# facebookresearch/gtn

Measured on AMD Instinct MI355X. Metric: CTC forward+backward losses/sec (T=1000, C=256), higher is better.
Workload: dtype f32; 1 GPU; BASELINE config C3: compose(ctc_target, emissions)+forwardScore CTC loss fwd+bwd, T=1000, C=256, U=100, batch=512 per GPU; global_batch=512, parallelism=dp1 (utterance sharding, all_gather of losses), rccl_ranks=0

## Files before the change

### gtn_amd/_capi.py

```python
import ctypes as C
import os

c_graph = C.c_void_p
c_graph_p = C.POINTER(C.c_void_p)
c_i32_p = C.POINTER(C.c_int)
c_i64_p = C.POINTER(C.c_int64)
c_u8_p = C.POINTER(C.c_uint8)
c_f32_p = C.POINTER(C.c_float)

GRAD_FN = C.CFUNCTYPE(C.c_int, C.c_void_p, c_graph_p, C.c_int, c_graph)
CTX_FREE = C.CFUNCTYPE(None, C.c_void_p)

OK, INVALID_ARGUMENT, LOGIC_ERROR, RUNTIME_ERROR, OUT_OF_RANGE, DEVICE_ERROR = range(6)

_SIGS = {
    "gtnx_set_device": [C.c_int],
    "gtnx_get_device": [c_i32_p],
    "gtnx_set_stream": [C.c_void_p],
    "gtnx_compose_mode": [C.c_int, C.POINTER(C.c_int)],
    "gtnx_synchronize": [],
    "gtnx_memory_stats": [C.POINTER(C.c_uint64), C.POINTER(C.c_uint64)],
    "gtnx_empty_cache": [],
    "gtnx_reclaim": [],
    "gtnx_graph_create": [C.c_int, c_graph_p],
# ... 67 lines not shown
    "gtnx_viterbi_path_n": [c_graph_p, C.c_int, c_graph_p],
    "gtnx_items_n": [c_graph_p, C.c_int, C.c_void_p],
    "gtnx_items_device_n": [c_graph_p, C.c_int, C.c_void_p],
    "gtnx_grads_device_n": [c_graph_p, C.c_int, C.c_void_p, C.c_void_p],
    "gtnx_grads_bind_device_n": [c_graph_p, C.c_int, C.c_void_p, C.c_void_p],
    "gtnx_clone": [c_graph, C.c_int, c_graph_p],
    "gtnx_concat": [c_graph_p, C.c_int, c_graph_p],
    "gtnx_closure": [c_graph, c_graph_p],
    "gtnx_union": [c_graph_p, C.c_int, c_graph_p],
    "gtnx_batch_from_graphs": [c_graph_p, C.c_int, c_graph_p],
    "gtnx_batch_ctc_targets": [C.c_void_p, C.c_void_p, C.c_int, C.c_int, C.c_int, c_graph_p],
    "gtnx_batch_ctc_loss_step": [C.c_void_p, C.c_void_p, C.c_void_p, C.c_int, C.c_int, C.c_int, C.c_int, C.c_void_p,
                                 C.c_void_p, C.c_int, C.c_void_p],
    "gtnx_batch_ctc_loss_step_ok": [C.c_void_p, C.c_void_p, C.c_int, C.c_int, C.c_int, C.c_int, C.c_void_p, C.c_void_p,
                                    C.POINTER(C.c_int)],
    "gtnx_batch_asg_force_align": [C.c_void_p, C.c_void_p, C.c_int, c_graph, C.c_int, c_graph_p],
    "gtnx_batch_linear": [C.c_int, C.c_int, C.c_int, C.c_int, C.c_void_p, C.c_int, c_graph_p],
    "gtnx_batch_linear_rows": [C.c_int, C.c_int, C.c_int, C.c_void_p, C.c_int, C.c_void_p, C.c_int, c_graph_p],
    "gtnx_batch_destroy": [c_graph],
    "gtnx_batch_size": [c_graph, c_i32_p],
    "gtnx_batch_get": [c_graph, C.c_int, c_graph_p],
    "gtnx_batch_negate": [c_graph, c_graph_p],
    "gtnx_batch_add": [c_graph, c_graph, c_graph_p],
    "gtnx_batch_subtract": [c_graph, c_graph, c_graph_p],
    "gtnx_batch_subtract_into": [c_graph, c_graph, C.c_void_p, c_graph_p],
    "gtnx_batch_compose": [c_graph, c_graph, c_graph_p],
    "gtnx_batch_intersect": [c_graph, c_graph, c_graph_p],
    "gtnx_batch_forward_score": [c_graph, c_graph_p],
    "gtnx_batch_viterbi_score": [c_graph, c_graph_p],
    "gtnx_batch_viterbi_path": [c_graph, c_graph_p],
# ... 137 lines not shown
```

### gtn_amd/csrc/band_backward_body.inc

```
  constexpr int RNk = K >= 4 ? 4 : K;
  constexpr int NP = K / RNk;
  const BandPair P = GTNX_BAND_PAIR;
  const int T = P.T, C = P.C, NS = P.NS;
  extern __shared__ float lds[];
  const BandLds L = band_lds(C, K, NSmax, true);
  float* ering = lds + L.o_ering;
  float* aring = lds + L.o_aring;
  float* oring = lds + L.o_oring;
  int* snode = reinterpret_cast<int*>(lds + L.o_snode);
  const BandMisc M = band_misc<K>(lds, L);
  float* lser = M.lsep;
  const int CS = L.CS;
  const int wv = __builtin_amdgcn_readfirstlane(threadIdx.x >> 6);
  const bool sweeper = wv < 4;
  const int l = threadIdx.x & 63;
  const int nblocks = (T + K - 1) / K;
  const int nticks = nblocks + 5;
  const GTNX_G double* ao = P.aoff;
  const double z2 = uniform(ao[0]);
  const bool dead = !(z2 > double(DEADF));
  const float ds = uniform(P.delta[0]);
  const bool want_em = P.grad_em != nullptr;
  GTNX_TM_INIT(128);
  constexpr bool SPLIT = !BIG && K >= 2 && GTNX_BWD_SPLIT;
// ... 121 lines not shown
    const bool have = all != 0.0f && !dead_r;
    const float f = have ? ds * __builtin_amdgcn_rcpf(all) : 1.0f;
    if ((l & 15) == 15 && (STEADY || (l >> 4) < rows)) {
      if (P.hot >= 0) {
        const float sm = dn_k * ex2(em_hot - ls_hot);
        const GTNX_G char* gb = reinterpret_cast<const GTNX_G char*>(P.grad_em + int64_t(T - c * K - K) * C);
        *reinterpret_cast<GTNX_G float*>(const_cast<GTNX_G char*>(gb) + unsigned(4 * R.go)) = (dead_r ? 0.0f : hotp * f) + sm;
      }
      rnorm_k[cg * K + (l >> 4)] = f;
    }
  };
  constexpr int NCS = 8 / K;
  struct DrainRegs {
    int s[NCS], e[NCS], n0[NCS], n1[NCS];
    float m0[NCS], m1[NCS];
    bool more_any;
  };
  auto drain_init = [&](DrainRegs& D, int hid) {
    const int* cls = reinterpret_cast<const int*>(oring);
#pragma unroll
    for (int q = 0; q < NCS; ++q) {
      const int cc = hid + q * BW;
      D.s[q] = D.e[q] = 0;
      if (cc < C && cc != P.hot) {
        D.s[q] = cls[cc];
        D.e[q] = cls[C + cc];
      }
      const int cnt = D.e[q] - D.s[q];
      D.n0[q] = cnt > 0 ? snode[D.s[q]] : 0;
      D.n1[q] = cnt > 1 ? snode[D.s[q] + 1] : 0;
      D.m0[q] = cnt > 0 ? 1.0f : 0.0f;
      D.m1[q] = cnt > 1 ? 1.0f : 0.0f;
    }
    D.more_any = false;
#pragma unroll
    for (int q = 0; q < NCS; ++q) D.more_any = D.more_any || __builtin_amdgcn_ballot_w64(D.e[q] - D.s[q] > 2) != 0;
  };
  auto drain_rows = [&](const DrainRegs& D, int hid, int c, int cg , auto full_tag, auto dead_tag, auto r0_tag, auto r1_tag) {
    constexpr bool FULL = decltype(full_tag)::value;
    constexpr bool DEADU = decltype(dead_tag)::value;
    constexpr int R0 = decltype(r0_tag)::value, R1 = decltype(r1_tag)::value;
    const int rows = FULL ? K : rows_of_k(c);
    const float* ob = oring + cg * K * NSmax;
    const float* eb = ering + ge_of(c) * K * CS;
    const float* lb = lser + cg * K;
    const float* fb = rnorm_k + cg * K;
    GTNX_G float* dst = P.grad_em + int64_t(T - 1 - c * K) * C;
#pragma unroll
    for (int q = 0; q < NCS; ++q) {
      if (q > 0 && q * BW >= C) break;
      const int cc = hid + q * BW;
      const bool mine = cc < C && cc != P.hot;
      float p0[K], p1[K], e[K], ls[K], f[K];
#pragma unroll
      for (int r = R0; r < R1; ++r) {
        if constexpr (!DEADU) {
          p0[r] = ob[r * NSmax + D.n0[q]];
          p1[r] = ob[r * NSmax + D.n1[q]];
        }
        e[r] = eb[r * CS + min(cc, C - 1)];
      }
      if constexpr (K == 4) {
        const gtnx_f4 l4 = *reinterpret_cast<const gtnx_f4*>(lb), f4 = *reinterpret_cast<const gtnx_f4*>(fb);
        ls[0] = l4.x, ls[1] = l4.y, ls[2] = l4.z, ls[3] = l4.w;
        f[0] = f4.x, f[1] = f4.y, f[2] = f4.z, f[3] = f4.w;
      } else {
#pragma unroll
        for (int r = R0; r < R1; ++r) {
          ls[r] = lb[r];
          f[r] = fb[r];
        }
      }
      float sum[K];
      if constexpr (!DEADU) {
#pragma unroll
      for (int r = R0; r < R1; ++r) sum[r] = p0[r] * D.m0[q] + p1[r] * D.m1[q];
      }
      if (!DEADU && D.more_any) {
        for (int i = D.s[q] + 2; i < D.e[q]; ++i) {
          const float* o = ob + snode[i];
#pragma unroll
          for (int r = R0; r < R1; ++r) sum[r] += o[r * NSmax];
        }
      }
      float val[K];
#pragma unroll
      for (int r = R0; r < R1; ++r) {
        const float sm = dn_k * ex2(e[r] - ls[r]);
        val[r] = DEADU ? sm : sum[r] * f[r] + sm;
      }
      if (mine) {
#pragma unroll
        for (int r = R0; r < R1; ++r) {
          if (FULL || r < rows) {
            GTNX_G float* row = dst - int64_t(r) * C;
            row[cc] = val[r];
          }
        }
      }
    }
  };
  auto drain_block = [&](const DrainRegs& D, int hid, int c, int cg, auto r0_tag, auto r1_tag) {
    if (!want_em || c >= nblocks) return;
    if (dead) drain_rows(D, hid, c, cg, std::false_type{}, std::true_type{}, r0_tag, r1_tag);
    else if (c * K + K <= T) drain_rows(D, hid, c, cg, std::true_type{}, std::false_type{}, r0_tag, r1_tag);
    else drain_rows(D, hid, c, cg, std::false_type{}, std::false_type{}, r0_tag, r1_tag);
  };
  constexpr int KH = SPLIT ? K / 2 : K;

  if (sweeper) {
#ifndef GTNX_BWD_SWEEP_PRIO
#define GTNX_BWD_SWEEP_PRIO 1
#endif
    __builtin_amdgcn_s_setprio(GTNX_BWD_SWEEP_PRIO);
    const int w = wv;
    const int lag = 3 - w;
    const int m0 = threadIdx.x * NPL;
    NodeRegs<NPL> g;
    load_nodes<NPL, true>(P, m0, g);
    float b[NPL], post[NPL], acc[3][NPL];
    const double Ahi = uniform(ao[1 + (T >> P.lgrn) * 4 + w]);
// ... 14 lines not shown
    }
    float* bnd_own = M.bndr + (4 - w) * 4 * K * 2;
    const float* bnd_prev = M.bndr + (3 - w) * 4 * K * 2;
    double* off_own = M.offr + (4 - w) * 16;
    const double* off_prev = M.offr + (3 - w) * 16;
    if (threadIdx.x < 8 * K) M.bndr[threadIdx.x] = NEGF;
    if (threadIdx.x < 16) M.offr[threadIdx.x] = 0.0;
    if (l == 0) off_own[0] = 0.0;
    lds_barrier();
    lds_barrier();
    RowSumRegs rsr;
    if constexpr (!SPLIT && !RS4) rowsum_init(rsr);
    float gscale = ds;
    int bm5 = ring_start(-lag, NBE), bm7 = ring_start(-lag, NBG), rm7 = ring_start(RS4 ? -5 : -4, NBG);
    lds_barrier();
    auto tick = [&](int tau, auto steady_tag) {
      constexpr bool STEADY = decltype(steady_tag)::value;
      GTNX_TM(0);
      if constexpr (RS4) {
#ifndef GTNX_EXP_NO_GSCALE
        if (GRADG && want_em && (STEADY || (tau >= 5 && (tau - 5) * K + K <= T))) gscale = rnorm_k[rm7 * K + w];
#endif
      } else if constexpr (!SPLIT) {
#ifndef GTNX_EXP_NO_ROWSUM
        if (STEADY || tau >= 4) {
          const float fr = rowsum_do(rsr, tau - 4, rm7, w, steady_tag);
#ifndef GTNX_EXP_NO_GSCALE
          if (fr != 0.0f) gscale = fr;
#endif
        }
// ... 134 lines not shown
        }
        if (NPL == 1 ? l < 2 : l == 0) {
#pragma unroll
          for (int i = 0; i < K; ++i)
            if (FULL || i < rows) {
              float* bp = bnd_own + ((beta & 3) * K + i) * 2;
              if (NPL == 1) {
                bp[l] = qh[i][0];
              } else {
                bp[0] = qh[i][0];
                bp[1] = qh[i][NPL - 1];
              }
            }
        }
      };
      if constexpr (STEADY) {
        block(std::true_type{});
      } else if (beta >= 0 && beta < nblocks && !dead) {
        if (beta * K + K <= T) block(std::true_type{});
        else block(std::false_type{});
      }
      GTNX_TM(5);
      lds_barrier();
      GTNX_TM(6);
      GTNX_TM_TICK();
    };
    {
      const int s0 = min(RS4 ? 5 : 4, nticks), s1 = dead ? s0 : max(s0, min(nticks, T / K + lag));
      auto step_rings = [&]() { ring_step(bm5, NBE), ring_step(bm7, NBG), ring_step(rm7, NBG); };
      int tau = 0;
      for (; tau < s0; ++tau, step_rings()) tick(tau, std::false_type{});
      for (; tau < s1; ++tau, step_rings()) tick(tau, std::true_type{});
      for (; tau < nticks; ++tau, step_rings()) tick(tau, std::false_type{});
    }
    GTNX_TM_DUMP();
    if (GRADG && P.grad_fixed) {
#pragma unroll
      for (int j = 0; j < NPL; ++j)
#pragma unroll
        for (int k = 0; k < 3; ++k)
          if (g.ao[k][j] >= 0) P.grad_fixed[g.ao[k][j]] = dead ? 0.0f : acc[k][j];
    }
  } else if (wv < 8) {
    const bool soft = P.delta_norm != nullptr && P.rowlse != nullptr;
    lds_barrier();
    if constexpr (!BIG) {
      const int h = wv - 4, q = h & 1;
      auto rows_of = [&](int c) { return c < nblocks ? min(K, T - c * K) : 0; };
      auto tlo_of = [&](int c) { return T - c * K - rows_of(c); };
      DrainRegs dr_s;
      const int hid_s = threadIdx.x - BW;
      auto drain_upper = [&](int tau) {
        if constexpr (SPLIT) {
          if (tau >= 5) drain_block(dr_s, hid_s, tau - 5, (tau - 5) % NBG, std::integral_constant<int, KH>{}, std::integral_constant<int, K>{});
        }
      };
      if (h < 2) {
        Stage<16, 64> se;
        if constexpr (VEC) se.init_offsets(C, CS, K, l);
        auto issue_em = [&](int c, auto steady_tag) {
          constexpr bool ST = decltype(steady_tag)::value;
          const int rows = ST ? K : rows_of(c);
          se.template issue<VEC>(P.em + int64_t(T - c * K - rows) * C, rows * C, l);
        };
        auto land_em = [&](int c, auto steady_tag) {
          constexpr bool ST = decltype(steady_tag)::value;
          const int rows = ST ? K : rows_of(c);
          se.settle_all();
          GTNX_TM(4);
// ... 5 lines not shown
              const f2v lo = f2v{v4.x, v4.y} * LOG2E, hi = f2v{v4.z, v4.w} * LOG2E;
              *reinterpret_cast<gtnx_f4*>(eb + o) = gtnx_f4{fmaxf(lo.x, NEGF), fmaxf(lo.y, NEGF), fmaxf(hi.x, NEGF), fmaxf(hi.y, NEGF)};
            });
          } else {
            se.template each<false>(rows * C, C, l, [&](int, int, int r, int col, gtnx_f4 v4) {
              eb[(rows - 1 - r) * CS + col] = em2(v4.x);
            });
          }
        };
        issue_em(q, std::false_type{});
        land_em(q, std::false_type{});
        issue_em(q + 2, std::false_type{});
        RowSum4Regs rs4;
        if constexpr (RS4) rowsum4_init(rs4);
        lds_barrier();
        if constexpr (SPLIT) drain_init(dr_s, hid_s);
        lds_barrier();
        int r7 = ring_start(-4, NBG);
        auto tick = [&](int tau, auto steady_tag) {
          constexpr bool ST = decltype(steady_tag)::value;
          GTNX_TM(0);
#ifndef GTNX_EXP_NO_STAGE
          if (((tau + 2) & 1) == q) {
            land_em(tau + 2, steady_tag);
            GTNX_TM(1);
            issue_em(tau + 4, steady_tag);
            GTNX_TM(2);
          } else if constexpr (RS4) {
#ifndef GTNX_EXP_NO_ROWSUM
            if (ST || tau >= 4) rowsum4_do(rs4, tau - 4, r7, steady_tag);
#endif
// ... 31 lines not shown
          const int rows = ST ? K : rows_of(c);
          sa.settle_all();
          asm volatile("" : "+v"(lse_s), "+v"(af_s));
          if (rows <= 0) return;
          float* ab = aring + c5 * K * NSmax;
          sa.each_vec(rows * NS, (K - rows) * NSmax, l, [&](int, int o, gtnx_f4 v4) { *reinterpret_cast<gtnx_f4*>(ab + o) = v4; });
          if (l < rows) lser[c7 * K + rows - 1 - l] = lse_s;
          if (l < 4 * rows) M.aofr[(c5 * K) * 4 + l] = af_s;
        };
        issue_rest(q, std::false_type{});
        if (q == 0) {
          land_rest(0, 0, 0, std::false_type{});
          issue_rest(2, std::false_type{});
        }
        lds_barrier();
        if constexpr (SPLIT) drain_init(dr_s, hid_s);
        lds_barrier();
        int s5 = ring_start(1, NBE), s7 = ring_start(1, NBG);
        auto tick = [&](int tau, auto steady_tag) {
          GTNX_TM(0);
#ifndef GTNX_EXP_NO_STAGE
          if (((tau + 1) & 1) == q) {
            land_rest(tau + 1, s5, s7, steady_tag);
            GTNX_TM(1);
            issue_rest(tau + 3, steady_tag);
            GTNX_TM(2);
          }
#endif
          drain_upper(tau);
          GTNX_TM(3);
          lds_barrier();
// ... 86 lines not shown
    GTNX_TM_DUMP();
    }
  } else {
    const int hid = threadIdx.x - 2 * BW;
    const bool soft = P.delta_norm != nullptr && P.rowlse != nullptr;
    int* cls = reinterpret_cast<int*>(oring);
    for (int c = hid; c < 2 * C; c += BW) cls[c] = 0;
    lds_barrier();
    for (int i = hid; i < P.n_lab; i += BW) {
      const int lab = P.slab[i];
      snode[i] = P.snode[i];
      if (i == 0 || P.slab[i - 1] != lab) cls[lab] = i;
      if (i == P.n_lab - 1 || P.slab[i + 1] != lab) cls[C + lab] = i + 1;
    }
    lds_barrier();
    DrainRegs dr;
    drain_init(dr, hid);
    RowSumRegs rsr;
    if constexpr (SPLIT) rowsum_init(rsr);
    const int dw = wv - 8;
    lds_barrier();
    int d7 = ring_start(-5, NBG);
    for (int tau = 0; tau < nticks; ++tau, ring_step(d7, NBG)) {
      GTNX_TM(0);
#ifndef GTNX_EXP_NO_DRAIN
      if (tau >= 5) drain_block(dr, hid, tau - 5, d7, std::integral_constant<int, 0>{}, std::integral_constant<int, KH>{});
#endif
      if constexpr (SPLIT) {
        if (tau >= 4) rowsum_do(rsr, tau - 4, (tau - 4) % NBG, dw, std::false_type{});
      }
      GTNX_TM(3);
      lds_barrier();
      GTNX_TM(6);
      GTNX_TM_TICK();
    }
    GTNX_TM_DUMP();
  }
```

### gtn_amd/csrc/band_forward_body.inc

```
#ifndef GTNX_FWD_SHIFT_ROWS
#define GTNX_FWD_SHIFT_ROWS 4
#endif
  constexpr int RNk = K >= GTNX_FWD_SHIFT_ROWS ? GTNX_FWD_SHIFT_ROWS : (K >= 4 ? 4 : K);
  constexpr int NP = K / RNk;
  constexpr int D = 8 / K > GTNX_FWD_DEPTH ? 8 / K : GTNX_FWD_DEPTH;
  const BandPair P = GTNX_BAND_PAIR;
  const int T = P.T, C = P.C, NS = P.NS;
  extern __shared__ float lds[];
  const BandLds L = band_lds(C, K, NSmax, false);
  float* ering = lds + L.o_ering;
  const BandMisc M = band_misc<K>(lds, L);
  const int CS = L.CS;
  const int wv = __builtin_amdgcn_readfirstlane(threadIdx.x >> 6);
  const bool sweeper = wv < 4;
  const int l = threadIdx.x & 63;
  const int nblocks = (T + K - 1) / K;
  const int nticks = nblocks + 3;
  GTNX_TM_INIT(0);

  if (sweeper) {
    __builtin_amdgcn_s_setprio(1);
    const int w = wv;
    const int m0 = threadIdx.x * NPL;
    NodeRegs<NPL> g;
// ... 16 lines not shown
    const double* off_prev = M.offr + w * 16;
    if (threadIdx.x < 8 * K) M.bndr[threadIdx.x] = NEGF;
    if (threadIdx.x < 16) M.offr[threadIdx.x] = 0.0;
    if (l == 0) {
      P.aoff[1 + w] = 0.0;
      off_own[0] = 0.0;
    }
    if (NPL == 1) {
      if (l >= 62) bnd_own[63 - l] = a[0];
    } else if (l == 63) {
      bnd_own[0] = a[NPL - 1];
      bnd_own[1] = a[0];
    }
    lds_barrier();
    int bm5 = ((-w % NBE) + NBE) % NBE;
    for (int tau = 0; tau < nticks; ++tau, bm5 = bm5 + 1 == NBE ? 0 : bm5 + 1) {
      GTNX_TM(0);
      const int beta = tau - w;
      auto block = [&](auto full_tag) {
        constexpr bool FULL = decltype(full_tag)::value;
        const int t0 = beta * K, rows = FULL ? K : min(K, T - t0);
        const float* eb = ering + bm5 * K * CS;
        float ev[K][NPL], bv1[K], bv2[K];
        double offp[NP + 1];
#pragma unroll
        for (int i = 0; i < K; ++i) {
#pragma unroll
#ifdef GTNX_EXP_NOCONFLICT
          for (int j = 0; j < NPL; ++j) ev[i][j] = eb[i * CS + l * NPL + j];
#else
          for (int j = 0; j < NPL; ++j) ev[i][j] = eb[i * CS + g.lab[j]];
// ... 298 lines not shown
```

### gtn_amd/csrc/batch.cpp

```cpp
#include "batch.h"

#include <algorithm>
#include <atomic>
#include <cstdlib>
#include <cstring>
#include <limits>
#include <unordered_map>
#include <unordered_set>

namespace gtnx {

namespace {

std::atomic<uint64_t> g_batch_seq{1};

struct CompMode {
  int old;
  CompMode() : old(compose_mode_hint(2)) {}
  ~CompMode() { compose_mode_hint(old); }
};

BatchP make_batch(Batch::Kind k, int n, bool cg) {
  auto b = std::make_shared<Batch>();
  b->kind = k;
  b->n = n;
  b->calc_grad = cg;
  return b;
}

// ... 540 lines not shown
  d.aoff = arena->as<double>(o_aoff);
  d.rowlse = arena->as<float>(o_lse);
  d.score = arena->as<float>(o_score);
  d.norm = arena->as<float>(o_norm);
  d.em_stride = int64_t(T) * C;
  d.rec_stride = int64_t(rec_stride);
  d.alpha_stride = int64_t(alpha_stride);
  d.aoff_stride = int64_t(aoff_stride);
  d.o_flags = int(o_flags);
  d.o_snode = int(o_snode);
  d.o_slab = int(o_slab);
  d.T = T;
  d.C = C;
  d.blank = blank;
  d.lgrn = band_forward_lgrn(C);
  {
    GTNX_PROF("band_forward_score_grad", bytes);
    launch_ctc_step(d, n, max_ns, target_grad, rt.stream());
  }
}


BatchP batch_asg_force_align(const int* labels, const int* lengths, int n, Graph& transitions, int n_labels) {
  if (n < 0) throw_invalid("[gtnx_batch_asg_force_align] negative batch size");
  if (transitions.num_nodes() != int64_t(n_labels) + 1 || transitions.num_arcs() != int64_t(n_labels) * (n_labels + 1))
    throw_invalid("[gtnx_batch_asg_force_align] the transitions graph must have the asgTransitions(N) layout");
  BatchP b = make_batch(Batch::CTC_TARGETS, n, transitions.calc_grad());
  b->fal = true;
  b->trans = transitions;
  b->trans_labels = n_labels;
// ... 499 lines not shown
    std::shared_ptr<PendingCopy> pend = ch.w_pend;
    std::unique_lock<std::mutex> pend_lock;
    bool fuse_copy = false;
    if (pend && !pend->done.load(std::memory_order_acquire)) {
      pend_lock = std::unique_lock<std::mutex>(pend->mu);
      fuse_copy = !pend->done.load(std::memory_order_relaxed) && pend->device == rt.device();
      const size_t A = size_t(T) * size_t(C);
      for (int b = 0; b < n && fuse_copy; ++b) fuse_copy = pend->src_of(ch.w_dev + size_t(b) * A) != nullptr;
      fuse_copy = fuse_copy && pend->segs.size() == size_t(n);
      if (!fuse_copy) {
        pend_lock.unlock();
        pend->settle();
      }
    }
    int64_t goff_run = 0;
    for (int b = 0; b < n; ++b) {
      BandPair& p = op->pairs[size_t(b)];
      p = BandPair{};
      const int U = fx.lab_off[size_t(b) + 1] - fx.lab_off[size_t(b)];
      const size_t N = fx.fal ? size_t(U) + 1 : size_t(2 * U + 1);
      char* base = fx.rec_mem->as<char>(fx.rec_off[size_t(b)]);
      p.nodes = reinterpret_cast<BandNode*>(base);
      base += align_up(sizeof(BandNode) * N, 64);
      p.nflags = reinterpret_cast<uint8_t*>(base);
      base += align_up(N, 64);
      p.snode = reinterpret_cast<int*>(base);
      base += align_up(4 * N, 64);
      p.slab = reinterpret_cast<int*>(base);
      p.n_lab = fx.fal ? U : int(N);
      p.w = fx.fal ? fx.rec_mem->as<float>(fx.w_off[size_t(b)]) : nullptr;
      p.em = ch.w_dev + size_t(b) * size_t(T) * size_t(C);
      p.N = int(N);
      p.T = ch.rows_of(b);
      p.C = C;
      p.NS = band_row_stride(p.N, band_npl(p.N));
      p.alpha = op->arena->as<float>(ao[size_t(b)]);
      p.aoff = op->arena->as<double>(oo[size_t(b)]);
      p.score = op->arena->as<float>(4 * size_t(b));
      if (want_norm) {
        p.norm = op->arena->as<float>(o_norm + 4 * size_t(b));
        p.rowlse = op->arena->as<float>(o_lse + 4 * size_t(b) * size_t(T));
      }
      p.hot = (!fx.fal && U + 1 >= 8) ? fx.blank : -1;
      p.lgrn = band_forward_lgrn(C);
      p.bidx = b;
      p.goff = goff_run;
      goff_run += int64_t(fx.elem_size(b));
      BandPair q = p;
      if (fuse_copy) {
        q.em = static_cast<const float*>(pend->src_of(p.em));
        q.em_copy = const_cast<float*>(p.em);
      }
      tab.push_back({BandLaunchKey{C, band_npl(q.N), fx.fal ? 0 : 1, 0, band_vec_ok(q)}, q});
      abytes += 4.0 * p.T * C + 4.0 * double(p.T + 1) * p.NS + (fuse_copy ? 4.0 * T * C : 0.0);
    }
    band_launch(tab, false, "band_forward_score", abytes, fuse_copy ? nullptr : &op->fwd_table);
    if (fuse_copy) pend->done.store(true, std::memory_order_release);
    if (want_norm) {
      ch.nc_mem = op->arena;
// ... 296 lines not shown
```

### gtn_amd/csrc/capi.cpp

```cpp
#include <atomic>
#include <chrono>
#include <condition_variable>
#include <cstdlib>
#include <cstring>
#include <mutex>
#include <string>
#include <vector>

#include "batch.h"
#include "lm_graph.h"
#include "ops.h"
#include "ops_internal.h"
#include "region.h"

#define GTNX_API extern "C" __attribute__((visibility("default")))

using namespace gtnx;

namespace {
thread_local std::string g_err;

gtnx_status_t fail(gtnx_status_t s, const std::string& m) {
  g_err = m;
  return s;
// ... 745 lines not shown
}
GTNX_API gtnx_status_t gtnx_batch_ctc_loss_step(const void* emissions, const int* labels, const int* lengths, int n, int T,
                                                int C, int blank, void* loss, void* grad, int target_grad,
                                                void* target_grad_dev) {
  return guard([&] {
    batch_ctc_loss_step(emissions, labels, lengths, n, T, C, blank, loss, grad, target_grad != 0, target_grad_dev);
  });
}
GTNX_API gtnx_status_t gtnx_batch_ctc_loss_step_ok(const int* labels, const int* lengths, int n, int T, int C, int blank,
                                                   const void* emissions, const void* grad, int* ok) {
  return guard([&] {
    if (!ok) throw_invalid("[gtnx_batch_ctc_loss_step_ok] null result pointer");
    *ok = ctc_step_fused_ok(labels, lengths, n, T, C, blank, emissions, grad) ? 1 : 0;
  });
}
GTNX_API gtnx_status_t gtnx_batch_asg_force_align(const int* labels, const int* lengths, int n, gtnx_graph_t transitions,
                                                  int n_labels, gtnx_batch_t* out) {
  return guard([&] { *out = HB(batch_asg_force_align(labels, lengths, n, G(transitions), n_labels)); });
}
GTNX_API gtnx_status_t gtnx_batch_linear(int n, int M, int N, int cg, const void* dev, int borrow, gtnx_batch_t* out) {
  return guard([&] { *out = HB(batch_linear(n, M, N, cg != 0, dev, borrow != 0)); });
}
GTNX_API gtnx_status_t gtnx_batch_linear_rows(int n, int M, int N, const int* rows, int cg, const void* dev, int borrow,
                                             gtnx_batch_t* out) {
  return guard([&] { *out = HB(batch_linear(n, M, N, cg != 0, dev, borrow != 0, rows)); });
}
GTNX_API gtnx_status_t gtnx_batch_destroy(gtnx_batch_t b) {
  return guard([&] {
    auto* p = reinterpret_cast<BatchP*>(b);
    if (!p) return;
// ... 477 lines not shown
```

### gtn_amd/csrc/ctc_step.hip

```cpp
#include <hip/hip_runtime.h>

#include <algorithm>
#include <atomic>
#include <stdexcept>
#include <type_traits>

#include "kernels.h"

namespace gtnx {
namespace {

#include "band_device.inc"

__device__ float g_ctc_step_seeds[2] = {-1.0f, 1.0f};

__device__ __forceinline__ BandPair step_pair(const CtcStepDesc& d, int b, const gtnx_i4 e) {
  BandPair P;
  const int U = e.y, N = 2 * U + 1;
  GTNX_G char* rec = reinterpret_cast<GTNX_G char*>(d.rec) + int64_t(b) * d.rec_stride;
  P.nodes = reinterpret_cast<const GTNX_G BandNode*>(rec);
  P.nflags = reinterpret_cast<const GTNX_G uint8_t*>(rec + d.o_flags);
  P.snode = reinterpret_cast<const GTNX_G int*>(rec + d.o_snode);
  P.slab = reinterpret_cast<const GTNX_G int*>(rec + d.o_slab);
  P.w = nullptr;
// ... 5 lines not shown
  P.rowlse = reinterpret_cast<GTNX_G float*>(d.rowlse) + int64_t(b) * d.T;
  P.norm = reinterpret_cast<GTNX_G float*>(d.norm) + b;
  P.delta = (const GTNX_G float*)g_ctc_step_seeds;
  P.delta_norm = (const GTNX_G float*)(g_ctc_step_seeds + 1);
  P.grad_em = reinterpret_cast<GTNX_G float*>(d.grad) + int64_t(b) * d.em_stride;
  P.grad_fixed = d.tgrad ? reinterpret_cast<GTNX_G float*>(d.tgrad) + e.w : nullptr;
  P.N = N;
  P.T = e.z;
  P.C = d.C;
  P.NS = (N + 3) & ~3;
  P.hot = U + 1 >= 8 ? d.blank : -1;
  P.lgrn = d.lgrn;
  P.n_lab = N;
  P.bidx = b;
  P.goff = e.w;
  return P;
}

__device__ __forceinline__ BandPair uniform_pair(const BandPair& s) {
  constexpr int NW = int(sizeof(BandPair) / 4);
  static_assert(sizeof(BandPair) % 4 == 0, "a pair is whole words");
  const int* src = reinterpret_cast<const int*>(&s);
  int w[NW];
#pragma unroll
  for (int i = 0; i < NW; ++i) w[i] = __builtin_amdgcn_readfirstlane(src[i]);
  BandPair P;
  __builtin_memcpy(&P, w, sizeof(BandPair));
  return P;
}

// ... 116 lines not shown
```

### gtn_amd/csrc/kernels.h

```cpp
#pragma once

#include <hip/hip_runtime.h>

#include <cstdint>

#include <atomic>
#include <cstdint>
struct gtnx_first_on_device {
  std::atomic<uint64_t>& done;
  uint64_t bit;
  bool first;
  explicit gtnx_first_on_device(std::atomic<uint64_t>& d) : done(d) {
    int dev = 0;
    (void)hipGetDevice(&dev);
    bit = uint64_t(1) << (dev & 63);
    first = !(done.load(std::memory_order_acquire) & bit);
  }
  gtnx_first_on_device(const gtnx_first_on_device&) = delete;
  ~gtnx_first_on_device() {
    if (first) done.fetch_or(bit, std::memory_order_acq_rel);
  }
  explicit operator bool() const { return first; }
};

// ... 343 lines not shown
  GTNX_G float* alpha;
  GTNX_G double* aoff;
  GTNX_G float* score;
  GTNX_G float* norm;
  GTNX_G float* rowlse;
  const GTNX_G float* delta;
  const GTNX_G float* delta_norm;
  GTNX_G float* grad_em;
  GTNX_G float* grad_fixed;
  int N, T, C, NS;
  int hot;
  int lgrn;
  int n_lab;
  int bidx;
  int64_t goff;
};
struct BandPatch {
  int on;
  int M;
  const GTNX_G float* delta;
  const GTNX_G float* delta_norm;
  GTNX_G float* rowlse;
  GTNX_G float* grad_em;
  GTNX_G float* grad_fixed;
  int64_t A;
};
struct BandDecode {
  const GTNX_G BandNode* nodes;
  const GTNX_G uint8_t* nflags;
  const GTNX_G float* w;
  const GTNX_G float* em;
// ... 102 lines not shown
  const GTNX_G int* stage;
  const GTNX_G int* labels;
  const GTNX_G float* em;
  GTNX_G float* grad;
  GTNX_G float* loss;
  GTNX_G float* tgrad;
  GTNX_G char* rec;
  GTNX_G float* alpha;
  GTNX_G double* aoff;
  GTNX_G float* rowlse;
  GTNX_G float* score;
  GTNX_G float* norm;
  int64_t em_stride, rec_stride, alpha_stride, aoff_stride;
  int o_flags, o_snode, o_slab;
  int T, C, blank, lgrn;
};
int band_block_rows(int C, int max_NS, bool backward);
bool ctc_step_cell(int C, int max_NS);
void launch_ctc_step(const CtcStepDesc& d, int n, int max_NS, bool gradg, hipStream_t st);
struct AsgFalArgs {
  const GTNX_G int* labels;
  const GTNX_G float* trans_w;
  GTNX_G BandNode* nodes;
  GTNX_G uint8_t* nflags;
  GTNX_G int* snode;
  GTNX_G int* slab;
  GTNX_G float* w;
  GTNX_G int* arc_map;
  int U, pad;
};
// ... 326 lines not shown
```

### include/gtn_amd.h

```cpp
#ifndef GTN_AMD_H
#define GTN_AMD_H

#include <stddef.h>
#include <stdint.h>

#ifdef __cplusplus
extern "C" {
#endif

typedef int gtnx_status_t;
#define GTNX_OK 0
#define GTNX_INVALID_ARGUMENT 1
#define GTNX_LOGIC_ERROR 2
#define GTNX_RUNTIME_ERROR 3
#define GTNX_OUT_OF_RANGE 4
#define GTNX_DEVICE_ERROR 5

typedef struct gtnx_graph_s* gtnx_graph_t;

#define GTNX_EPSILON (-1)

const char* gtnx_last_error(void);
const char* gtnx_version(void);
const char* gtnx_backend(void);
// ... 99 lines not shown

gtnx_status_t gtnx_clone(gtnx_graph_t g, int projection , gtnx_graph_t* out);
gtnx_status_t gtnx_concat(const gtnx_graph_t* g, int n, gtnx_graph_t* out);
gtnx_status_t gtnx_closure(gtnx_graph_t g, gtnx_graph_t* out);
gtnx_status_t gtnx_union(const gtnx_graph_t* g, int n, gtnx_graph_t* out);
gtnx_status_t gtnx_remove(gtnx_graph_t g, int ilabel, int olabel, gtnx_graph_t* out);

typedef struct gtnx_batch_s* gtnx_batch_t;
gtnx_status_t gtnx_batch_from_graphs(const gtnx_graph_t* g, int n, gtnx_batch_t* out);
gtnx_status_t gtnx_batch_ctc_targets(const int* labels, const int* lengths, int n, int blank, int calc_grad,
                                     gtnx_batch_t* out);
gtnx_status_t gtnx_batch_ctc_loss_step(const void* emissions, const int* labels, const int* lengths, int n, int T, int C,
                                       int blank, void* loss, void* grad, int target_grad, void* target_grad_dev);
gtnx_status_t gtnx_batch_ctc_loss_step_ok(const int* labels, const int* lengths, int n, int T, int C, int blank,
                                          const void* emissions, const void* grad, int* ok);
gtnx_status_t gtnx_batch_asg_force_align(const int* labels, const int* lengths, int n, gtnx_graph_t transitions,
                                         int n_labels, gtnx_batch_t* out);
gtnx_status_t gtnx_batch_linear(int n, int M, int N, int calc_grad, const void* device_weights, int borrow,
                                gtnx_batch_t* out);
gtnx_status_t gtnx_batch_linear_rows(int n, int M, int N, const int* rows, int calc_grad, const void* device_weights,
                                     int borrow, gtnx_batch_t* out);
gtnx_status_t gtnx_batch_destroy(gtnx_batch_t b);
gtnx_status_t gtnx_batch_size(gtnx_batch_t b, int* out);
gtnx_status_t gtnx_batch_get(gtnx_batch_t b, int i, gtnx_graph_t* out);
gtnx_status_t gtnx_batch_negate(gtnx_batch_t a, gtnx_batch_t* out);
gtnx_status_t gtnx_batch_add(gtnx_batch_t a, gtnx_batch_t b, gtnx_batch_t* out);
gtnx_status_t gtnx_batch_subtract(gtnx_batch_t a, gtnx_batch_t b, gtnx_batch_t* out);
gtnx_status_t gtnx_batch_subtract_into(gtnx_batch_t a, gtnx_batch_t b, void* items_device, gtnx_batch_t* out);
gtnx_status_t gtnx_batch_compose(gtnx_batch_t a, gtnx_batch_t b, gtnx_batch_t* out);
gtnx_status_t gtnx_batch_intersect(gtnx_batch_t a, gtnx_batch_t b, gtnx_batch_t* out);
// ... 150 lines not shown
```

Baseline: 1.010 million losses/s.

## Skip provably dead CTC band blocks via reachability live window; specialize drain loop

Computes, per wavefront, the range of time blocks whose CTC lattice states can be reached from a start state and can still reach an accept state. Blocks outside that window are skipped and only their boundary, offset and gradient rings are filled with neutral values. This applies to both the forward and backward band kernels. The backward gradient drain also gets specialized loops that precompute store offsets, fix the set count and the extra-arc path at compile time, and use an fma. The risk is correctness if the reachability bounds are off by one, plus some extra register pressure from the per-row offsets.

```diff
diff --git a/gtn_amd/_capi.py b/gtn_amd/_capi.py
--- a/gtn_amd/_capi.py
+++ b/gtn_amd/_capi.py
@@ -105,6 +105,7 @@
                                  C.c_void_p, C.c_int, C.c_void_p],
     "gtnx_batch_ctc_loss_step_ok": [C.c_void_p, C.c_void_p, C.c_int, C.c_int, C.c_int, C.c_int, C.c_void_p, C.c_void_p,
                                     C.POINTER(C.c_int)],
+    "gtnx_batch_band_live_blocks": [C.c_int, C.c_int, C.c_int, C.c_int, C.c_int, C.c_int, C.c_int, C.POINTER(C.c_int)],
     "gtnx_batch_asg_force_align": [C.c_void_p, C.c_void_p, C.c_int, c_graph, C.c_int, c_graph_p],
     "gtnx_batch_linear": [C.c_int, C.c_int, C.c_int, C.c_int, C.c_void_p, C.c_int, c_graph_p],
     "gtnx_batch_linear_rows": [C.c_int, C.c_int, C.c_int, C.c_void_p, C.c_int, C.c_void_p, C.c_int, c_graph_p],
diff --git a/gtn_amd/csrc/band_backward_body.inc b/gtn_amd/csrc/band_backward_body.inc
--- a/gtn_amd/csrc/band_backward_body.inc
+++ b/gtn_amd/csrc/band_backward_body.inc
@@ -159,12 +159,15 @@
   struct DrainRegs {
     int s[NCS], e[NCS], n0[NCS], n1[NCS];
     float m0[NCS], m1[NCS];
+    int so[NCS][K];
     bool more_any;
   };
-  auto drain_init = [&](DrainRegs& D, int hid) {
+  auto drain_base = [&](int c) { return reinterpret_cast<const GTNX_G char*>(P.grad_em) + (int64_t(T) - int64_t(c) * K - K) * C * 4; };
+  auto drain_init = [&](DrainRegs& D, int hid, auto nsets_tag) {
+    constexpr int NSETS = decltype(nsets_tag)::value;
     const int* cls = reinterpret_cast<const int*>(oring);
 #pragma unroll
-    for (int q = 0; q < NCS; ++q) {
+    for (int q = 0; q < NSETS; ++q) {
       const int cc = hid + q * BW;
       D.s[q] = D.e[q] = 0;
       if (cc < C && cc != P.hot) {
@@ -176,12 +179,19 @@
       D.n1[q] = cnt > 1 ? snode[D.s[q] + 1] : 0;
       D.m0[q] = cnt > 0 ? 1.0f : 0.0f;
       D.m1[q] = cnt > 1 ? 1.0f : 0.0f;
+#pragma unroll
+      for (int r = 0; r < K; ++r) {
+        D.so[q][r] = 4 * ((K - 1 - r) * C + min(cc, C - 1));
+        settle(D.so[q][r]);
+      }
     }
     D.more_any = false;
 #pragma unroll
-    for (int q = 0; q < NCS; ++q) D.more_any = D.more_any || __builtin_amdgcn_ballot_w64(D.e[q] - D.s[q] > 2) != 0;
-  };
-  auto drain_rows = [&](const DrainRegs& D, int hid, int c, int cg , auto full_tag, auto dead_tag, auto r0_tag, auto r1_tag) {
+    for (int q = 0; q < NSETS; ++q) D.more_any = D.more_any || __builtin_amdgcn_ballot_w64(D.e[q] - D.s[q] > 2) != 0;
+  };
+  auto drain_rows = [&](DrainRegs& D, int hid, int c, int cg , const GTNX_G char* gb, auto nsets_tag, auto more_tag, auto full_tag, auto dead_tag, auto r0_tag, auto r1_tag) {
+    constexpr int NSETS = decltype(nsets_tag)::value;
+    constexpr int MORE = decltype(more_tag)::value;
     constexpr bool FULL = decltype(full_tag)::value;
     constexpr bool DEADU = decltype(dead_tag)::value;
     constexpr int R0 = decltype(r0_tag)::value, R1 = decltype(r1_tag)::value;
@@ -190,9 +200,8 @@
     const float* eb = ering + ge_of(c) * K * CS;
     const float* lb = lser + cg * K;
     const float* fb = rnorm_k + cg * K;
-    GTNX_G float* dst = P.grad_em + int64_t(T - 1 - c * K) * C;
-#pragma unroll
-    for (int q = 0; q < NCS; ++q) {
+#pragma unroll
+    for (int q = 0; q < NSETS; ++q) {
       if (q > 0 && q * BW >= C) break;
       const int cc = hid + q * BW;
       const bool mine = cc < C && cc != P.hot;
@@ -221,7 +230,7 @@
 #pragma unroll
       for (int r = R0; r < R1; ++r) sum[r] = p0[r] * D.m0[q] + p1[r] * D.m1[q];
       }
-      if (!DEADU && D.more_any) {
+      if (!DEADU && MORE != 0 && (MORE == 2 || D.more_any)) {
         for (int i = D.s[q] + 2; i < D.e[q]; ++i) {
           const float* o = ob + snode[i];
 #pragma unroll
@@ -231,25 +240,31 @@
       float val[K];
 #pragma unroll
       for (int r = R0; r < R1; ++r) {
-        const float sm = dn_k * ex2(e[r] - ls[r]);
-        val[r] = DEADU ? sm : sum[r] * f[r] + sm;
+        const float x = ex2(e[r] - ls[r]);
+        if constexpr (DEADU) {
+          val[r] = dn_k * x;
+        } else {
+          const float ps = sum[r] * f[r];
+          val[r] = __builtin_fmaf(dn_k, x, ps);
+        }
       }
       if (mine) {
 #pragma unroll
         for (int r = R0; r < R1; ++r) {
           if (FULL || r < rows) {
-            GTNX_G float* row = dst - int64_t(r) * C;
-            row[cc] = val[r];
+            settle(D.so[q][r]);
+            *reinterpret_cast<GTNX_G float*>(const_cast<GTNX_G char*>(gb) + unsigned(D.so[q][r])) = val[r];
           }
         }
       }
     }
   };
-  auto drain_block = [&](const DrainRegs& D, int hid, int c, int cg, auto r0_tag, auto r1_tag) {
+  auto drain_block = [&](DrainRegs& D, int hid, int c, int cg, const GTNX_G char* gb, auto nsets_tag, auto r0_tag, auto r1_tag) {
     if (!want_em || c >= nblocks) return;
-    if (dead) drain_rows(D, hid, c, cg, std::false_type{}, std::true_type{}, r0_tag, r1_tag);
-    else if (c * K + K <= T) drain_rows(D, hid, c, cg, std::true_type{}, std::false_type{}, r0_tag, r1_tag);
-    else drain_rows(D, hid, c, cg, std::false_type{}, std::false_type{}, r0_tag, r1_tag);
+    constexpr std::integral_constant<int, 1> more_tag{};
+    if (dead) drain_rows(D, hid, c, cg, gb, nsets_tag, more_tag, std::false_type{}, std::true_type{}, r0_tag, r1_tag);
+    else if (c * K + K <= T) drain_rows(D, hid, c, cg, gb, nsets_tag, more_tag, std::true_type{}, std::false_type{}, r0_tag, r1_tag);
+    else drain_rows(D, hid, c, cg, gb, nsets_tag, more_tag, std::false_type{}, std::false_type{}, r0_tag, r1_tag);
   };
   constexpr int KH = SPLIT ? K / 2 : K;
 
@@ -294,6 +309,12 @@
     float gscale = ds;
     int bm5 = ring_start(-lag, NBE), bm7 = ring_start(-lag, NBG), rm7 = ring_start(RS4 ? -5 : -4, NBG);
     lds_barrier();
+    int blo, bhi;
+    {
+      const int wlo = w * 64 * NPL, whi = ((P.wstart || P.waccept) ? min(wlo + 64 * NPL, P.N) : wlo + 64 * NPL) - 1;
+      const int s_max = P.wstart ? P.wstart - 1 : BAND_ALL_LIVE, a_min = P.waccept ? P.waccept - 1 : -BAND_ALL_LIVE;
+      band_bwd_live_blocks(wlo, whi, s_max, a_min, T, K, &blo, &bhi);
+    }
     auto tick = [&](int tau, auto steady_tag) {
       constexpr bool STEADY = decltype(steady_tag)::value;
       GTNX_TM(0);
@@ -458,10 +479,43 @@
             }
         }
       };
+      auto skip_block = [&]() {
+        const int v0 = beta * K, rows = min(K, T - v0);
+#pragma unroll
+        for (int q = 1; q <= NP; ++q) {
+          if (q * RNk - 1 < rows) {
+            if (w < 3) bsum = off_prev[(beta * NP + q) & 15];
+            if (l == 0) off_own[((v0 + q * RNk) / RNk) & 15] = bsum;
+          }
+        }
+        if (want_em && m0 < NSmax) {
+          float* ob = oring + bm7 * K * NSmax + m0;
+#pragma unroll
+          for (int i = 0; i < K; ++i)
+            if (i < rows) {
+#pragma unroll
+              for (int j = 0; j < NPL; ++j) ob[i * NSmax + j] = 0.0f;
+            }
+        }
+        if (NPL == 1 ? l < 2 : l == 0) {
+#pragma unroll
+          for (int i = 0; i < K; ++i)
+            if (i < rows) {
+              float* bp = bnd_own + ((beta & 3) * K + i) * 2;
+              if (NPL == 1) {
+                bp[l] = NEGF;
+              } else {
+                bp[0] = NEGF;
+                bp[1] = NEGF;
+              }
+            }
+        }
+      };
       if constexpr (STEADY) {
         block(std::true_type{});
       } else if (beta >= 0 && beta < nblocks && !dead) {
-        if (beta * K + K <= T) block(std::true_type{});
+        if (beta < blo || beta > bhi) skip_block();
+        else if (beta * K + K <= T) block(std::true_type{});
         else block(std::false_type{});
       }
       GTNX_TM(5);
@@ -471,10 +525,11 @@
     };
     {
       const int s0 = min(RS4 ? 5 : 4, nticks), s1 = dead ? s0 : max(s0, min(nticks, T / K + lag));
+      const int sa = max(s0, min(s1, blo + lag)), sb = max(sa, min(s1, bhi + lag + 1));
       auto step_rings = [&]() { ring_step(bm5, NBE), ring_step(bm7, NBG), ring_step(rm7, NBG); };
       int tau = 0;
-      for (; tau < s0; ++tau, step_rings()) tick(tau, std::false_type{});
-      for (; tau < s1; ++tau, step_rings()) tick(tau, std::true_type{});
+      for (; tau < sa; ++tau, step_rings()) tick(tau, std::false_type{});
+      for (; tau < sb; ++tau, step_rings()) tick(tau, std::true_type{});
       for (; tau < nticks; ++tau, step_rings()) tick(tau, std::false_type{});
     }
     GTNX_TM_DUMP();
@@ -496,7 +551,7 @@
       const int hid_s = threadIdx.x - BW;
       auto drain_upper = [&](int tau) {
         if constexpr (SPLIT) {
-          if (tau >= 5) drain_block(dr_s, hid_s, tau - 5, (tau - 5) % NBG, std::integral_constant<int, KH>{}, std::integral_constant<int, K>{});
+          if (tau >= 5) drain_block(dr_s, hid_s, tau - 5, (tau - 5) % NBG, drain_base(tau - 5), std::integral_constant<int, NCS>{}, std::integral_constant<int, KH>{}, std::integral_constant<int, K>{});
         }
       };
       if (h < 2) {
@@ -532,7 +587,7 @@
         RowSum4Regs rs4;
         if constexpr (RS4) rowsum4_init(rs4);
         lds_barrier();
-        if constexpr (SPLIT) drain_init(dr_s, hid_s);
+        if constexpr (SPLIT) drain_init(dr_s, hid_s, std::integral_constant<int, NCS>{});
         lds_barrier();
         int r7 = ring_start(-4, NBG);
         auto tick = [&](int tau, auto steady_tag) {
@@ -594,7 +649,7 @@
           issue_rest(2, std::false_type{});
         }
         lds_barrier();
-        if constexpr (SPLIT) drain_init(dr_s, hid_s);
+        if constexpr (SPLIT) drain_init(dr_s, hid_s, std::integral_constant<int, NCS>{});
         lds_barrier();
         int s5 = ring_start(1, NBE), s7 = ring_start(1, NBG);
         auto tick = [&](int tau, auto steady_tag) {
@@ -711,25 +766,45 @@
       if (i == P.n_lab - 1 || P.slab[i + 1] != lab) cls[C + lab] = i + 1;
     }
     lds_barrier();
-    DrainRegs dr;
-    drain_init(dr, hid);
-    RowSumRegs rsr;
-    if constexpr (SPLIT) rowsum_init(rsr);
-    const int dw = wv - 8;
-    lds_barrier();
-    int d7 = ring_start(-5, NBG);
-    for (int tau = 0; tau < nticks; ++tau, ring_step(d7, NBG)) {
-      GTNX_TM(0);
+    auto drain_loop = [&](auto nsets_tag) {
+      DrainRegs dr;
+      drain_init(dr, hid, nsets_tag);
+      RowSumRegs rsr;
+      if constexpr (SPLIT) rowsum_init(rsr);
+      const int dw = wv - 8;
+      lds_barrier();
+      int d7 = ring_start(-5, NBG);
+      const GTNX_G char* gb = drain_base(-5);
+      const int64_t gstep = int64_t(K) * C * 4;
+      auto tick = [&](int tau, auto more_tag) {
+        constexpr int MORE = decltype(more_tag)::value;
+        GTNX_TM(0);
 #ifndef GTNX_EXP_NO_DRAIN
-      if (tau >= 5) drain_block(dr, hid, tau - 5, d7, std::integral_constant<int, 0>{}, std::integral_constant<int, KH>{});
-#endif
-      if constexpr (SPLIT) {
-        if (tau >= 4) rowsum_do(rsr, tau - 4, (tau - 4) % NBG, dw, std::false_type{});
-      }
-      GTNX_TM(3);
-      lds_barrier();
-      GTNX_TM(6);
-      GTNX_TM_TICK();
-    }
+        if constexpr (MORE != 1)
+          drain_rows(dr, hid, tau - 5, d7, gb, nsets_tag, more_tag, std::true_type{}, std::false_type{}, std::integral_constant<int, 0>{}, std::integral_constant<int, KH>{});
+        else if (tau >= 5)
+          drain_block(dr, hid, tau - 5, d7, gb, nsets_tag, std::integral_constant<int, 0>{}, std::integral_constant<int, KH>{});
+#endif
+        if constexpr (SPLIT) {
+          if (tau >= 4) rowsum_do(rsr, tau - 4, (tau - 4) % NBG, dw, std::false_type{});
+        }
+        GTNX_TM(3);
+        lds_barrier();
+        GTNX_TM(6);
+        GTNX_TM_TICK();
+      };
+      const int s0 = min(5, nticks), s1 = (dead || !want_em) ? s0 : max(s0, min(nticks, T / K + 5));
+      auto step = [&]() { ring_step(d7, NBG), gb -= gstep; };
+      int tau = 0;
+      for (; tau < s0; ++tau, step()) tick(tau, std::integral_constant<int, 1>{});
+      if (dr.more_any) {
+        for (; tau < s1; ++tau, step()) tick(tau, std::integral_constant<int, 2>{});
+      } else {
+        for (; tau < s1; ++tau, step()) tick(tau, std::integral_constant<int, 0>{});
+      }
+      for (; tau < nticks; ++tau, step()) tick(tau, std::integral_constant<int, 1>{});
+    };
+    if (NCS == 1 || C <= BW) drain_loop(std::integral_constant<int, 1>{});
+    else drain_loop(std::integral_constant<int, NCS>{});
     GTNX_TM_DUMP();
   }
diff --git a/gtn_amd/csrc/band_forward_body.inc b/gtn_amd/csrc/band_forward_body.inc
--- a/gtn_amd/csrc/band_forward_body.inc
+++ b/gtn_amd/csrc/band_forward_body.inc
@@ -54,7 +54,55 @@
     }
     lds_barrier();
     int bm5 = ((-w % NBE) + NBE) % NBE;
-    for (int tau = 0; tau < nticks; ++tau, bm5 = bm5 + 1 == NBE ? 0 : bm5 + 1) {
+    int tau = 0;
+    {
+      const int wlo = w * 64 * NPL, whi = (P.wstart ? min(wlo + 64 * NPL, P.N) : wlo + 64 * NPL) - 1;
+      const int s_max = P.wstart ? P.wstart - 1 : BAND_ALL_LIVE;
+      const int tlive = min(nticks, w + band_fwd_first_live_block(wlo, whi, s_max, T, K));
+      for (; tau < tlive; ++tau, bm5 = bm5 + 1 == NBE ? 0 : bm5 + 1) {
+        const int beta = tau - w;
+        if (beta >= 0) {
+          const int t0 = beta * K, rows = min(K, T - t0);
+#pragma unroll
+          for (int q = 1; q <= NP; ++q) {
+            if (q * RNk - 1 < rows) {
+              if (w > 0) off = off_prev[(beta * NP + q) & 15];
+              if (l == 0) {
+                const int p = (t0 + q * RNk) / RNk;
+                off_own[p & 15] = off;
+                P.aoff[1 + p * 4 + w] = off;
+              }
+            }
+          }
+          const GTNX_G char* const brow = arow;
+          arow += int64_t(NS) * 4 * rows;
+          if (writer) {
+#pragma unroll
+            for (int i = 0; i < K; ++i)
+              if (i < rows) {
+                const GTNX_G char* ri = brow + int64_t(NS) * 4 * (i + 1);
+#pragma unroll
+                for (int j = 0; j < NPL; ++j) *reinterpret_cast<GTNX_G float*>(const_cast<GTNX_G char*>(ri) + (aoffb + 4u * j)) = NEGF;
+              }
+          }
+          if (NPL == 1 ? l >= 62 : l == 63) {
+#pragma unroll
+            for (int i = 0; i < K; ++i)
+              if (i < rows) {
+                float* bp = bnd_own + ((((beta & 3) * K + i + 1) & (4 * K - 1))) * 2;
+                if (NPL == 1) {
+                  bp[63 - l] = NEGF;
+                } else {
+                  bp[0] = NEGF;
+                  bp[1] = NEGF;
+                }
+              }
+          }
+        }
+        lds_barrier();
+      }
+    }
+    for (; tau < nticks; ++tau, bm5 = bm5 + 1 == NBE ? 0 : bm5 + 1) {
       GTNX_TM(0);
       const int beta = tau - w;
       auto block = [&](auto full_tag) {
diff --git a/gtn_amd/csrc/batch.cpp b/gtn_amd/csrc/batch.cpp
--- a/gtn_amd/csrc/batch.cpp
+++ b/gtn_amd/csrc/batch.cpp
@@ -13,6 +13,11 @@
 namespace {
 
 std::atomic<uint64_t> g_batch_seq{1};
+
+bool band_live_window_on() {
+  const char* sw = std::getenv("GTNX_BAND_LIVE_WINDOW");
+  return !(sw && sw[0] == '0' && sw[1] == 0);
+}
 
 struct CompMode {
   int old;
@@ -583,6 +588,7 @@
   d.C = C;
   d.blank = blank;
   d.lgrn = band_forward_lgrn(C);
+  d.live_window = band_live_window_on() ? 1 : 0;
   {
     GTNX_PROF("band_forward_score_grad", bytes);
     launch_ctc_step(d, n, max_ns, target_grad, rt.stream());
@@ -1112,6 +1118,7 @@
       }
     }
     int64_t goff_run = 0;
+    const bool live_window = band_live_window_on();
     for (int b = 0; b < n; ++b) {
       BandPair& p = op->pairs[size_t(b)];
       p = BandPair{};
@@ -1141,6 +1148,10 @@
       }
       p.hot = (!fx.fal && U + 1 >= 8) ? fx.blank : -1;
       p.lgrn = band_forward_lgrn(C);
+      if (!fx.fal && live_window) {
+        p.wstart = 1 + 0;
+        p.waccept = 1 + (N >= 2 ? int(N) - 2 : 0);
+      }
       p.bidx = b;
       p.goff = goff_run;
       goff_run += int64_t(fx.elem_size(b));
diff --git a/gtn_amd/csrc/capi.cpp b/gtn_amd/csrc/capi.cpp
--- a/gtn_amd/csrc/capi.cpp
+++ b/gtn_amd/csrc/capi.cpp
@@ -783,6 +783,15 @@
     *ok = ctc_step_fused_ok(labels, lengths, n, T, C, blank, emissions, grad) ? 1 : 0;
   });
 }
+GTNX_API gtnx_status_t gtnx_batch_band_live_blocks(int lo, int hi, int s_max, int a_min, int T, int k_forward, int k_backward,
+                                             int* out) {
+  return guard([&] {
+    if (!out) throw_invalid("[gtnx_batch_band_live_blocks] null result pointer");
+    if (T < 1 || k_forward < 1 || k_backward < 1) throw_invalid("[gtnx_batch_band_live_blocks] T and the block sizes must be positive");
+    out[0] = band_fwd_first_live_block(lo, hi, s_max, T, k_forward);
+    band_bwd_live_blocks(lo, hi, s_max, a_min, T, k_backward, &out[1], &out[2]);
+  });
+}
 GTNX_API gtnx_status_t gtnx_batch_asg_force_align(const int* labels, const int* lengths, int n, gtnx_graph_t transitions,
                                                   int n_labels, gtnx_batch_t* out) {
   return guard([&] { *out = HB(batch_asg_force_align(labels, lengths, n, G(transitions), n_labels)); });
diff --git a/gtn_amd/csrc/ctc_step.hip b/gtn_amd/csrc/ctc_step.hip
--- a/gtn_amd/csrc/ctc_step.hip
+++ b/gtn_amd/csrc/ctc_step.hip
@@ -43,6 +43,8 @@
   P.n_lab = N;
   P.bidx = b;
   P.goff = e.w;
+  P.wstart = d.live_window ? 1 + 0 : 0;
+  P.waccept = d.live_window ? 1 + (N >= 2 ? N - 2 : 0) : 0;
   return P;
 }
 
diff --git a/gtn_amd/csrc/kernels.h b/gtn_amd/csrc/kernels.h
--- a/gtn_amd/csrc/kernels.h
+++ b/gtn_amd/csrc/kernels.h
@@ -381,7 +381,35 @@
   int n_lab;
   int bidx;
   int64_t goff;
-};
+  int wstart, waccept;
+};
+#if defined(__HIP__)
+#define GTNX_HD __host__ __device__
+#else
+#define GTNX_HD
+#endif
+constexpr int BAND_ALL_LIVE = 1 << 29;
+GTNX_HD inline int band_fwd_first_live_block(int lo, int hi, int s_max, int T, int K) {
+  const int nblocks = (T + K - 1) / K;
+  if (hi < lo) return nblocks;
+  const int d = lo - s_max;
+  if (d <= 0) return 0;
+  if (2 * T < d) return nblocks;
+  return (d + 2 * K - 1) / (2 * K) - 1;
+}
+GTNX_HD inline void band_bwd_live_blocks(int lo, int hi, int s_max, int a_min, int T, int K, int* blo, int* bhi) {
+  const int nblocks = (T + K - 1) / K;
+  *blo = nblocks;
+  *bhi = -1;
+  if (hi < lo) return;
+  const int d = lo - s_max;
+  const int e = a_min - hi;
+  const int tF = d <= 2 ? 0 : (d + 1) / 2 - 1;
+  const int tB = e <= 2 ? T - 1 : T - (e + 1) / 2;
+  if (tF > T - 1 || tB < 0 || tB < tF) return;
+  *bhi = (T - 1 - tF) / K;
+  *blo = (T - tB + K - 1) / K - 1;
+}
 struct BandPatch {
   int on;
   int M;
@@ -514,6 +542,7 @@
   int64_t em_stride, rec_stride, alpha_stride, aoff_stride;
   int o_flags, o_snode, o_slab;
   int T, C, blank, lgrn;
+  int live_window, pad;
 };
 int band_block_rows(int C, int max_NS, bool backward);
 bool ctc_step_cell(int C, int max_NS);
diff --git a/include/gtn_amd.h b/include/gtn_amd.h
--- a/include/gtn_amd.h
+++ b/include/gtn_amd.h
@@ -137,6 +137,7 @@
                                        int blank, void* loss, void* grad, int target_grad, void* target_grad_dev);
 gtnx_status_t gtnx_batch_ctc_loss_step_ok(const int* labels, const int* lengths, int n, int T, int C, int blank,
                                           const void* emissions, const void* grad, int* ok);
+gtnx_status_t gtnx_batch_band_live_blocks(int lo, int hi, int s_max, int a_min, int T, int k_forward, int k_backward, int* out);
 gtnx_status_t gtnx_batch_asg_force_align(const int* labels, const int* lengths, int n, gtnx_graph_t transitions,
                                          int n_labels, gtnx_batch_t* out);
 gtnx_status_t gtnx_batch_linear(int n, int M, int N, int calc_grad, const void* device_weights, int borrow,
```

Result: no change. 1.001 million losses/s (-0.9%).
